# google-research/seed_rl

Hardware: NVIDIA H100
Metric: env-frames/sec (learner, device-timed) on synthetic 84x84x4 T=20 unrolls @1/2/4/8 H100 (higher is better)
Workload: dtype bf16x3 (fp32-faithful tensor-core contraction; activations stored as bf16 hi+lo pairs), f32 elsewhere

## Files before the change

seed_rl_b200/csrc/capi.cu:

```cuda
#include <vector>

#include "common.cuh"

namespace seedrl {
thread_local std::string g_last_error;
std::atomic<uint64_t> g_launch_count{0};
bool g_prof_on = false;
int g_conv_cat = PC_CONV_FWD;

struct ProfRec { int cat; cudaEvent_t e; };
static std::vector<ProfRec> g_prof;
static cudaEvent_t g_prof_start;

void prof_mark_(int cat, cudaStream_t st) {
  ProfRec r;
  r.cat = cat;
  cudaEventCreate(&r.e);
  cudaEventRecord(r.e, st);
  g_prof.push_back(r);
}
}

static const char* kProfNames[seedrl::PC_COUNT] = {
    "conv3x3_fwd", "conv3x3_dgrad", "conv3x3_wgrad", "maxpool", "sgemm", "lstm_pointwise",
    "vtrace_loss", "adam", "vtrace", "misc"};

extern "C" const char* seedrl_last_error(void) { return seedrl::g_last_error.c_str(); }
extern "C" int seedrl_abi_version(void) { return 1; }
extern "C" uint64_t seedrl_kernel_launch_count(void) {
  return seedrl::g_launch_count.load(std::memory_order_relaxed);
}

extern "C" int seedrl_profile_num_categories(void) { return seedrl::PC_COUNT; }
extern "C" const char* seedrl_profile_category_name(int i) {
// ... 34 lines not shown
```

seed_rl_b200/csrc/common.cuh:

```cuda
#pragma once
#include <cuda_runtime.h>
#include <stdint.h>
#include <stdio.h>

#include <atomic>
#include <string>

#include "../../include/seedrl_b200.h"

namespace seedrl {

extern thread_local std::string g_last_error;
extern std::atomic<uint64_t> g_launch_count;

inline int set_error(int code, const std::string& msg) {
  g_last_error = msg;
  return code;
}

#define SEEDRL_TRY(expr)                \
  do {                                  \
    const int rc__ = (expr);            \
    if (rc__ != SEEDRL_OK) return rc__; \
  } while (0)
// ... 24 lines not shown
  } while (0)

enum ProfCat { PC_CONV_FWD = 0, PC_CONV_DGRAD, PC_CONV_WGRAD, PC_POOL, PC_GEMM, PC_LSTM_PW,
               PC_LOSS, PC_ADAM, PC_VTRACE, PC_MISC, PC_COUNT };
extern bool g_prof_on;
extern int g_conv_cat;
void prof_mark_(int cat, cudaStream_t st);

inline void count_launch(int cat = PC_MISC, cudaStream_t st = 0) {
  g_launch_count.fetch_add(1, std::memory_order_relaxed);
  if (g_prof_on) prof_mark_(cat, st);
}

constexpr int kNumSMs = 132;

__host__ __device__ inline int ceil_div(int a, int b) { return (a + b - 1) / b; }
__host__ __device__ inline size_t ceil_div_sz(size_t a, size_t b) { return (a + b - 1) / b; }

__device__ __forceinline__ float warp_sum(float v) {
#pragma unroll
  for (int o = 16; o > 0; o >>= 1) v += __shfl_xor_sync(0xffffffffu, v, o);
  return v;
}
__device__ __forceinline__ float warp_max(float v) {
#pragma unroll
  for (int o = 16; o > 0; o >>= 1) v = fmaxf(v, __shfl_xor_sync(0xffffffffu, v, o));
  return v;
}

__device__ __forceinline__ float sigmoidf_(float x) { return 1.0f / (1.0f + expf(-x)); }
// ... 16 lines not shown
```

seed_rl_b200/csrc/conv_first.cu:

```cuda
#include <cuda.h>

#include <cstdlib>
#include <cstring>

#include "kernels.h"
#include "tc_common.cuh"

namespace seedrl {

constexpr int kFwThreads = 256;
constexpr int kFwCo = 16;
constexpr int kFwLanes = kFwThreads / kFwCo;

static inline int first_layer_cp(int c) { return c <= 4 ? 4 : (c <= 8 ? 8 : 16); }
static inline int fw_rows_per_band(int cp) { return cp == 16 ? 4 : 6; }
static inline size_t fw_pixels_8b(int cp, int rb, int W) { return ((size_t)(2 * rb + 3) * (W + 2) * (cp / 4) + 1) & ~(size_t)1; }
static inline size_t fw_smem(int cp, int rb, int W) {
  const int wo = (W + 1) / 2;
  return fw_pixels_8b(cp, rb, W) * 8 + (size_t)rb * wo * kFwCo * 5;
}

struct FirstWgradArgs {
  int N, H, W, C, Ho, Wo, pt, pl;
  int Lpp, PWp, RHp;
// ... 446 lines not shown
  constexpr int KT = 3 * (CP == 16 ? 48 : 4 * CP);
  const int N = a.N, H = a.H, W = a.W;
  const size_t raw_stride = TMA ? (((size_t)(2 * ROWS + 3) * W * 4) + 127) / 128 * 128 : 0;
  const size_t smem = (size_t)(CP == 16 ? 2 : 1) * (MAXB * 128 + 2 * (W + 2) + 8) * 16 +
                      (size_t)MAXB * 128 * kCpOutStride * 4 + 128 + KT * 32 * 2 + 16 * 4 + 64 + 128 + 2 * raw_stride;
  static bool attr = false;
  if (!attr) {
    SEEDRL_CUDA(cudaFuncSetAttribute(conv0pool_kernel<ROWS, CP, TMA>, cudaFuncAttributeMaxDynamicSharedMemorySize,
                                     112 * 1024));
    attr = true;
  }
  if (smem > 112 * 1024) return set_error(SEEDRL_ERR_INVALID_ARGUMENT, "conv0pool: image too wide");
  CUtensorMap tm;
  memset(&tm, 0, sizeof(tm));
  if (TMA) {
    typedef CUresult (*EncodeTiledFn)(CUtensorMap*, CUtensorMapDataType, cuuint32_t, void*, const cuuint64_t*,
                                      const cuuint64_t*, const cuuint32_t*, const cuuint32_t*, CUtensorMapInterleave,
                                      CUtensorMapSwizzle, CUtensorMapL2promotion, CUtensorMapFloatOOBfill);
    static EncodeTiledFn enc = nullptr;
    if (!enc) {
      void* q = nullptr;
      cudaDriverEntryPointQueryResult qr;
      if (cudaGetDriverEntryPoint("cuTensorMapEncodeTiled", &q, cudaEnableDefault, &qr) != cudaSuccess ||
          qr != cudaDriverEntryPointSuccess)
        return set_error(SEEDRL_ERR_INTERNAL, "cuTensorMapEncodeTiled is not available");
      enc = reinterpret_cast<EncodeTiledFn>(q);
    }
    const cuuint64_t gdim[3] = {(cuuint64_t)W, (cuuint64_t)H, (cuuint64_t)N};
    const cuuint64_t gstr[2] = {(cuuint64_t)W * 4, (cuuint64_t)H * W * 4};
    const cuuint32_t box[3] = {(cuuint32_t)W, (cuuint32_t)(2 * ROWS + 3), 1};
    const cuuint32_t estr[3] = {1, 1, 1};
    if (enc(&tm, CU_TENSOR_MAP_DATA_TYPE_UINT32, 3, const_cast<uint8_t*>(frames), gdim, gstr, box, estr,
            CU_TENSOR_MAP_INTERLEAVE_NONE, CU_TENSOR_MAP_SWIZZLE_NONE, CU_TENSOR_MAP_L2_PROMOTION_L2_128B,
            CU_TENSOR_MAP_FLOAT_OOB_FILL_NONE) != CUDA_SUCCESS)
      return set_error(SEEDRL_ERR_INTERNAL, "conv0pool: cuTensorMapEncodeTiled failed");
  }
  const int units = N * ((a.Ho + ROWS - 1) / ROWS);
  const int per_sm = ROWS == 2 ? 3 : 2;
  const int grid = units < per_sm * kNumSMs ? units : per_sm * kNumSMs;
  conv0pool_kernel<ROWS, CP, TMA><<<grid, kCpThreadsF, smem, st>>>(tm, a);
  count_launch(PC_CONV_FWD, st);
  SEEDRL_CHECK_LAUNCH();
// ... 23 lines not shown
```

seed_rl_b200/csrc/conv_planes.cu:

```cuda
#include <cuda.h>
#include <cuda_bf16.h>

#include <cstdio>
#include <cstdlib>

#include "kernels.h"
#include "tc_common.cuh"

namespace seedrl {

long long planes_positions(int N, int H, int W) {
  const long long Q = (long long)N * (H + 1) * (W + 2);
  return ((Q + 2 * (W + 2) + 2 + 256 + 127) / 128) * 128;
}
size_t planes_bytes(int N, int H, int W, int C) {
  return (size_t)planes_positions(N, H, W) * 16 * 2 * (C / 8);
}

typedef CUresult (*EncodeTiledFn)(CUtensorMap*, CUtensorMapDataType, cuuint32_t, void*, const cuuint64_t*,
                                  const cuuint64_t*, const cuuint32_t*, const cuuint32_t*,
                                  CUtensorMapInterleave, CUtensorMapSwizzle, CUtensorMapL2promotion,
                                  CUtensorMapFloatOOBfill);
static EncodeTiledFn encode_tiled_fn() {
  static EncodeTiledFn fn = nullptr;
  static bool tried = false;
  if (!tried) {
    tried = true;
    void* q = nullptr;
    cudaDriverEntryPointQueryResult qr;
    if (cudaGetDriverEntryPoint("cuTensorMapEncodeTiled", &q, cudaEnableDefault, &qr) == cudaSuccess &&
        qr == cudaDriverEntryPointSuccess)
      fn = reinterpret_cast<EncodeTiledFn>(q);
    (void)cudaGetLastError();
  }
  return fn;
}

static int g_chunk = 0;
int planes_chunk() {
  if (g_chunk == 0) {
    const char* e = getenv("SEEDRL_PLANES_CHUNK");
    g_chunk = e ? atoi(e) : 128;
    if (g_chunk != 16 && g_chunk != 32 && g_chunk != 64 && g_chunk != 128) g_chunk = 128;
  }
  return g_chunk;
}

static int make_plane_map(CUtensorMap* tm, const void* base, long long Lp, int planes, int shift,
                          int CH, int box_chunks, int box_planes) {
  EncodeTiledFn enc = encode_tiled_fn();
// ... 5 lines not shown
  const cuuint32_t box[3] = {(cuuint32_t)(2 * CH), (cuuint32_t)box_chunks, (cuuint32_t)box_planes};
  const cuuint32_t estr[3] = {1, 1, 1};
  void* addr = const_cast<char*>(reinterpret_cast<const char*>(base)) + (size_t)shift * 16;
  const CUresult r = enc(tm, CU_TENSOR_MAP_DATA_TYPE_UINT64, 3, addr, gdim, gstr, box, estr,
                         CU_TENSOR_MAP_INTERLEAVE_NONE, CU_TENSOR_MAP_SWIZZLE_NONE,
                         CU_TENSOR_MAP_L2_PROMOTION_L2_256B, CU_TENSOR_MAP_FLOAT_OOB_FILL_NONE);
  if (r != CUDA_SUCCESS) {
    char msg[128];
    snprintf(msg, sizeof msg, "cuTensorMapEncodeTiled failed (%d) Lp=%lld planes=%d shift=%d box=%dx%d", (int)r, Lp,
             planes, shift, box_chunks, box_planes);
    return set_error(SEEDRL_ERR_INTERNAL, msg);
  }
  return SEEDRL_OK;
}

__device__ __forceinline__ void mbar_expect_tx(uint64_t* bar, uint32_t bytes) {
  asm volatile("mbarrier.arrive.expect_tx.shared::cta.b64 _, [%0], %1;" ::"r"(smem_u32(bar)), "r"(bytes)
               : "memory");
}
__device__ __forceinline__ void tma_load_3d(void* dst, const CUtensorMap* tm, int c0, int c1, int c2,
                                            uint64_t* bar) {
  asm volatile(
      "cp.async.bulk.tensor.3d.shared::cluster.global.tile.mbarrier::complete_tx::bytes [%0], [%1, {%2, %3, %4}], [%5];" ::
          "r"(smem_u32(dst)),
      "l"(reinterpret_cast<uint64_t>(tm)), "r"(c0), "r"(c1), "r"(c2), "r"(smem_u32(bar))
      : "memory");
}
__device__ __forceinline__ float bf16lo(uint32_t w) { return __uint_as_float(w << 16); }
__device__ __forceinline__ float bf16hi(uint32_t w) { return __uint_as_float(w & 0xFFFF0000u); }

struct ConvpArgs {
  ConvGeom g;
  int Lp;
  int nch;
// ... 655 lines not shown
```

seed_rl_b200/csrc/gemm_tc_kernels.cu:

```cuda
#include <cstdlib>

#include "kernels.h"
#include "tc_common.cuh"

namespace seedrl {

constexpr int kGtThreads = 256;
constexpr int kGtBM = 128;
constexpr int kGtMaxBN = 128;

struct GemmTcParams {
  int M, N, K;
  const float* A; int lda;
  const float* B; int ldb;
  float* C; int ldc;
  float* ws;
  int BN;
  int kblocks_per_split;
  int vecA, vecB;
  GemmEpi e;
  int* error_flag;
  ConvGather cg;
};

// ... 43 lines not shown
      r.b = __ldg(src + 1);
    }
  }
  return r;
}
template <bool SPLIT>
__device__ __forceinline__ void store_unit(RawUnit r, bool relu, uint4* hi_dst, uint4* lo_dst) {
  if (relu) {
    r.a.x = fmaxf(r.a.x, 0.f); r.a.y = fmaxf(r.a.y, 0.f); r.a.z = fmaxf(r.a.z, 0.f); r.a.w = fmaxf(r.a.w, 0.f);
    r.b.x = fmaxf(r.b.x, 0.f); r.b.y = fmaxf(r.b.y, 0.f); r.b.z = fmaxf(r.b.z, 0.f); r.b.w = fmaxf(r.b.w, 0.f);
  }
  *hi_dst = pack8_bf16(r.a, r.b);
  if (SPLIT) *lo_dst = pack8_bf16(bf16_resid4(r.a), bf16_resid4(r.b));
}

template <int TA, int TB>
__device__ __forceinline__ void gemm_tc_mma(int bn, float* acc, uint64_t a, uint64_t b) {
  switch (bn) {
    case 16: Wgmma<16>::mma<TA, TB>(acc, a, b, 1u); break;
    case 32: Wgmma<32>::mma<TA, TB>(acc, a, b, 1u); break;
    case 48: Wgmma<48>::mma<TA, TB>(acc, a, b, 1u); break;
    case 64: Wgmma<64>::mma<TA, TB>(acc, a, b, 1u); break;
    case 80: Wgmma<80>::mma<TA, TB>(acc, a, b, 1u); break;
    case 96: Wgmma<96>::mma<TA, TB>(acc, a, b, 1u); break;
    case 112: Wgmma<112>::mma<TA, TB>(acc, a, b, 1u); break;
    default: Wgmma<128>::mma<TA, TB>(acc, a, b, 1u); break;
  }
}

template <bool TA, bool TB, bool SPLIT, int kGtBK, bool GATHER>
// ... 90 lines not shown
  {
    const int ld = BN + 4;
    float* tile = reinterpret_cast<float*>(smem_raw);
    const int w = (tid >> 5) & 3, l = tid & 31;
    const int r0 = wg * 64 + 16 * w + (l >> 2), c0 = 2 * (l & 3);
#pragma unroll
    for (int j = 0; j < kGtMaxBN / 8; ++j) {
      if (8 * j < BN) {
#pragma unroll
        for (int h = 0; h < 2; ++h)
          *reinterpret_cast<float2*>(tile + (size_t)(r0 + 8 * h) * ld + 8 * j + c0) =
              make_float2(acc[4 * j + 2 * h], acc[4 * j + 2 * h + 1]);
      }
    }
    __syncthreads();
    const bool partial = p.ws != nullptr;
    for (int i = tid; i < kGtBM * BN; i += kGtThreads) {
      const int r = i / BN, c = i - r * BN;
      const int gm = m0 + r, gn = n0 + c;
      if (gm < p.M && gn < p.N) {
        float x = tile[(size_t)r * ld + c];
        if (partial) {
          p.ws[((size_t)blockIdx.z * p.M + gm) * p.N + gn] = x;
        } else {
          if (p.e.bias) x += __ldg(p.e.bias + gn);
          if (p.e.relu) x = fmaxf(x, 0.f);
          if (p.e.mask) x = __ldg(p.e.mask + (size_t)gm * p.e.ldm + gn) > 0.f ? x : 0.f;
          float* cp = p.C + (size_t)gm * p.ldc + gn;
          *cp = p.e.accumulate ? *cp + x : x;
        }
      }
    }
  }
}

template <bool VEC>
__global__ void gemm_tc_reduce_kernel(int M, int N, int splits, const float* __restrict__ ws,
                                      float* __restrict__ C, int ldc, GemmEpi e) {
  constexpr int W = VEC ? 4 : 1;
  const int i = (blockIdx.x * blockDim.x + threadIdx.x) * W;
  if (i >= M * N) return;
  const int m = i / N, n = i - m * N;
  float x[W];
#pragma unroll
  for (int j = 0; j < W; ++j) x[j] = 0.f;
  const size_t plane = (size_t)M * N;
#pragma unroll 4
// ... 73 lines not shown

bool conv_gather_setup(const void* x, int u8, int N, int H, int W, int C, int K, int S, ConvGather* g) {
  const int Ho = (H - K) / S + 1, Wo = (W - K) / S + 1, KC = K * C;
  if (Ho < 2 || Wo < 2 || KC < 8 || (KC & 7)) return false;
  if ((long long)N * Ho * Wo >= (1ll << 31)) return false;
  if (u8 ? (((W * C) & 7) || ((S * C) & 7) || (reinterpret_cast<uintptr_t>(x) & 7))
         : ((C & 3) || (reinterpret_cast<uintptr_t>(x) & 15)))
    return false;
  g->x = x; g->u8 = u8; g->H = H; g->W = W; g->C = C; g->S = S; g->Ho = Ho; g->Wo = Wo; g->KC = KC;
  fast_div_setup((unsigned int)Wo, &g->wo_mul, &g->wo_sh);
  fast_div_setup((unsigned int)Ho, &g->ho_mul, &g->ho_sh);
  fast_div_setup((unsigned int)KC, &g->kc_mul, &g->kc_sh);
  return true;
}

int gemm_tc(bool ta, bool tb, int split, int M, int N, int K, const float* A, int lda, const float* B,
            int ldb, float* C, int ldc, const GemmEpi& e, float* ws, size_t ws_bytes, int* err,
            cudaStream_t st, const ConvGather* cg) {
  if (M <= 0 || N <= 0) return SEEDRL_OK;
  SEEDRL_CHECK_ARG(!cg || (!tb && ((ta ? M : K) & 7) == 0), "gathered operand: tb or a ragged kernel row");
  GemmTcParams p;
  if (cg) p.cg = *cg; else p.cg = ConvGather{};
  p.M = M; p.N = N; p.K = K; p.A = A; p.lda = lda; p.B = B; p.ldb = ldb; p.C = C; p.ldc = ldc;
  p.e = e; p.error_flag = err;
  const int n16 = ((N + 15) / 16) * 16;
  const int BK = g_gemm_bk;
  int bn = kGtMaxBN;
  if (bn > n16) bn = n16;
  const int nkb_all = ceil_div(K, BK);
  const int kb256 = 256 / BK;
  while (bn > 64 && ceil_div(M, kGtBM) * ceil_div(N, bn) * (nkb_all >= kb256 ? nkb_all / (kb256 / 2) : 1) < kNumSMs)
    bn >>= 1;
  p.BN = ((bn + 15) / 16) * 16;
// ... 5 lines not shown
  int splits = 1;
  static const int waves = getenv("SEEDRL_GEMM_WAVES") ? atoi(getenv("SEEDRL_GEMM_WAVES")) : 1;
  while (tiles * splits < waves * kNumSMs && nkb / (splits * 2) >= 128 / BK &&
         (size_t)(splits * 2) * M * N * sizeof(float) <= ws_bytes && ws)
    splits *= 2;
  p.kblocks_per_split = ceil_div(nkb, splits);
  splits = ceil_div(nkb, p.kblocks_per_split);
  p.ws = splits > 1 ? ws : nullptr;
  const int S = split ? 2 : 1;
  const size_t a_un = ta ? (size_t)(kGtBM / 8) * (BK + 1) : (size_t)(BK / 8) * (kGtBM + 1);
  const size_t b_un = tb ? (size_t)(BK / 8) * (p.BN + 1) : (size_t)(p.BN / 8) * (BK + 1);
  size_t smem = (size_t)2 * S * (a_un + b_un) * 16;
  const size_t epi = (size_t)kGtBM * (p.BN + 4) * 4;
  if (smem < epi) smem = epi;
  dim3 grid(ceil_div(N, p.BN), ceil_div(M, kGtBM), splits);
#define SEEDRL_GT_LAUNCH2(TA_, TB_, SP_, BK_, G_)                                               \
  do {                                                                                          \
    static bool attr = false;                                                                   \
    if (!attr) {                                                                                \
      SEEDRL_CUDA(cudaFuncSetAttribute(gemm_tc_kernel<TA_, TB_, SP_, BK_, G_>,                  \
                                       cudaFuncAttributeMaxDynamicSharedMemorySize, 200 * 1024)); \
      attr = true;                                                                              \
    }                                                                                           \
    gemm_tc_kernel<TA_, TB_, SP_, BK_, G_><<<grid, kGtThreads, smem, st>>>(p);                  \
  } while (0)
#define SEEDRL_GT_LAUNCH1(TA_, TB_, SP_, BK_)                                                   \
  do {                                                                                          \
    if (cg && !(TB_)) SEEDRL_GT_LAUNCH2(TA_, false, SP_, BK_, true);                            \
    else SEEDRL_GT_LAUNCH2(TA_, TB_, SP_, BK_, false);                                          \
  } while (0)
// ... 5 lines not shown
  } while (0)
  if (split) {
    if (!ta && !tb) SEEDRL_GT_LAUNCH(false, false, true);
    else if (ta && !tb) SEEDRL_GT_LAUNCH(true, false, true);
    else if (!ta && tb) SEEDRL_GT_LAUNCH(false, true, true);
    else SEEDRL_GT_LAUNCH(true, true, true);
  } else {
    if (!ta && !tb) SEEDRL_GT_LAUNCH(false, false, false);
    else if (ta && !tb) SEEDRL_GT_LAUNCH(true, false, false);
    else if (!ta && tb) SEEDRL_GT_LAUNCH(false, true, false);
    else SEEDRL_GT_LAUNCH(true, true, false);
  }
#undef SEEDRL_GT_LAUNCH
#undef SEEDRL_GT_LAUNCH1
#undef SEEDRL_GT_LAUNCH2
  count_launch(PC_GEMM, st);
  SEEDRL_CHECK_LAUNCH();
  if (splits > 1) {
    if ((N & 3) == 0 && splits >= 16)
      gemm_tc_reduce_wide_kernel<<<ceil_div(M * N / 4, 32), 256, 0, st>>>(M, N, splits, ws, C, ldc, e);
    else if ((N & 3) == 0)
      gemm_tc_reduce_kernel<true><<<ceil_div(M * N / 4, 256), 256, 0, st>>>(M, N, splits, ws, C, ldc, e);
    else
      gemm_tc_reduce_kernel<false><<<ceil_div(M * N, 256), 256, 0, st>>>(M, N, splits, ws, C, ldc, e);
    count_launch(PC_GEMM, st);
    SEEDRL_CHECK_LAUNCH();
  }
  return SEEDRL_OK;
}

}
```

seed_rl_b200/csrc/kernels.h:

```cpp
#pragma once
#include "common.cuh"

namespace seedrl {

enum { IN_F32 = 0, IN_RELU = 1, IN_U8 = 2 };

struct ConvGeom {
  int N, H, W;
  int PW;
  int RH;
  long long Q;
  unsigned int pw_mul, rh_mul;
  int pw_sh, rh_sh;
};

__host__ __device__ inline void fast_div_setup(unsigned int d, unsigned int* mul, int* sh) {
  int l = 1;
  while ((1u << l) < d) ++l;
  *mul = (unsigned int)(((1ULL << (31 + l)) + d - 1) / d);
  *sh = l - 1;
}
__host__ __device__ __forceinline__ unsigned int fast_div(unsigned int n, unsigned int mul, int sh) {
#ifdef __CUDA_ARCH__
  return __umulhi(n, mul) >> sh;
// ... 130 lines not shown
size_t gemm_tc_workspace_bytes();
struct ConvGather {
  const void* x;
  int u8;
  int H, W, C, S, Ho, Wo;
  int KC;
  unsigned int wo_mul, ho_mul, kc_mul;
  int wo_sh, ho_sh, kc_sh;
};
bool conv_gather_setup(const void* x, int u8, int N, int H, int W, int C, int K, int S, ConvGather* g);
void gemm_tc_set_gather(int on);
bool gemm_tc_gather_enabled();
int gemm_tc(bool ta, bool tb, int split, int M, int N, int K, const float* A, int lda, const float* B,
            int ldb, float* C, int ldc, const GemmEpi& e, float* ws, size_t ws_bytes, int* err,
            cudaStream_t st, const ConvGather* cg = nullptr);
int fill(size_t n, float* p, float v, cudaStream_t st);

int lstm_forward_tiled(int H, int T1, int B, const float* U, const uint8_t* done, float* z, const float* h0,
                       const float* c0, float* hs, float* cs, float* hp, unsigned int* counter, int* err,
                       cudaStream_t st);
int lstm_backward_tiled(int H, int T1, int B, const float* U, const uint8_t* done, const float* gates,
                        const float* cs, const float* c0, const float* dhs, float* dz, unsigned int* counter,
                        int* err, cudaStream_t st);

int lstm_forward_tc(int H, int T1, int B, const float* U, const uint8_t* done, float* z, const float* h0,
                    const float* c0, float* hs, float* cs, float* hp, unsigned int* counter, int* err,
                    cudaStream_t st);
int lstm_backward_tc(int H, int T1, int B, const float* U, const uint8_t* done, const float* gates,
                     const float* cs, const float* c0, const float* dhs, float* dz, unsigned int* counter,
                     int* err, cudaStream_t st);
// ... 3 lines not shown
```

seed_rl_b200/csrc/net.cu:

```cuda
#include "schedule.h"

namespace seedrl {

constexpr int kHidden = 256;

struct ConvLayer {
  int cin, cout;
  int w, b;
};
struct Stack {
  int hin, win, cin, c, hout, wout;
  ConvLayer conv, r00, r01, r10, r11;
};

}

struct seedrl_net {
  seedrl_net_config cfg;
  seedrl::ParamTable params;
  size_t logical_params;
  int p_base_w, p_base_b, p_pol_w, p_pol_b;
  seedrl::Core core;
  std::vector<seedrl::Stack> stacks;
  seedrl::StridedConv sh[2];
// ... 697 lines not shown
                                          const void* x, const float* dy, float* dw, float* db,
                                          float* partial, size_t partial_bytes,
                                          seedrl_stream_t stream) {
  return conv3x3_wgrad(cin, cout, in_mode, N, H, W, x, dy, dw, db, partial, partial_bytes,
                       (cudaStream_t)stream);
}
extern "C" int seedrl_debug_maxpool(int backward, int N, int H, int W, int C, const float* x_or_dy,
                                    float* y_or_dx, uint8_t* idx, seedrl_stream_t stream) {
  if (backward) return maxpool3s2_backward(N, H, W, C, x_or_dy, idx, y_or_dx, (cudaStream_t)stream);
  return maxpool3s2_forward(N, H, W, C, x_or_dy, y_or_dx, idx, (cudaStream_t)stream);
}
extern "C" int seedrl_debug_gemm_tc(int ta, int tb, int split, int M, int N, int K, const float* A, int lda,
                                    const float* B, int ldb, float* C, int ldc, const float* bias,
                                    const float* mask, int ldm, int relu, int accumulate, int a_relu,
                                    float* ws, size_t ws_bytes, int* error_flag, seedrl_stream_t stream) {
  SEEDRL_CHECK_ARG(M >= 1 && N >= 1 && K >= 1 && A && B && C, "bad arguments");
  GemmEpi e{bias, mask, ldm, relu, accumulate, a_relu};
  return gemm_tc(ta != 0, tb != 0, split, M, N, K, A, lda, B, ldb, C, ldc, e, ws, ws_bytes, error_flag,
                 (cudaStream_t)stream);
}

extern "C" int seedrl_debug_sgemm(int ta, int tb, int M, int N, int K, const float* A, int lda,
                                  const float* B, int ldb, float* C, int ldc, const float* bias,
                                  const float* mask, int ldm, int relu, int accumulate, int a_relu,
                                  seedrl_stream_t stream) {
  GemmEpi e{bias, mask, ldm, relu, accumulate, a_relu};
  return sgemm(ta != 0, tb != 0, M, N, K, A, lda, B, ldb, C, ldc, e, (cudaStream_t)stream);
}

extern "C" int seedrl_debug_set_gemm_gather(int on) {
  gemm_tc_set_gather(on);
  return SEEDRL_OK;
// ... 118 lines not shown
```

seed_rl_b200/csrc/tc_common.cuh:

```cuda
#pragma once
#include <cuda_bf16.h>
#include <stdint.h>

namespace seedrl {

__device__ __forceinline__ uint32_t smem_u32(const void* p) {
  return static_cast<uint32_t>(__cvta_generic_to_shared(p));
}

__device__ __forceinline__ bool elect_one() {
  uint32_t pred;
  asm volatile(
      "{\n\t.reg .pred P;\n\t"
      "elect.sync _|P, 0xffffffff;\n\t"
      "selp.u32 %0, 1, 0, P;\n\t}\n"
      : "=r"(pred));
  return pred != 0;
}

__device__ __forceinline__ uint64_t gmma_desc(uint32_t addr, uint32_t lbo_bytes, uint32_t sbo_bytes) {
  uint64_t d = 0;
  d |= (uint64_t)((addr & 0x3FFFFu) >> 4);
  d |= (uint64_t)((lbo_bytes >> 4) & 0x3FFFu) << 16;
  d |= (uint64_t)((sbo_bytes >> 4) & 0x3FFFu) << 32;
// ... 44 lines not shown
        "selp.u32 %0, 1, 0, p;\n\t}\n"
        : "=r"(done)
        : "r"(smem_u32(bar)), "r"(parity)
        : "memory");
    if (!done && ++spins > (1 << 22)) return false;
  }
  return true;
}
__device__ __forceinline__ void mbar_init(uint64_t* bar, int count) {
  asm volatile("mbarrier.init.shared::cta.b64 [%0], %1;" ::"r"(smem_u32(bar)), "r"(count));
}
__device__ __forceinline__ void mbar_arrive(uint64_t* bar) {
  asm volatile("{\n\t.reg .b64 st;\n\tmbarrier.arrive.shared::cta.b64 st, [%0];\n\t}\n" ::"r"(smem_u32(bar))
               : "memory");
}

template <>
struct Wgmma<16> {
  template <int TA, int TB>
  __device__ __forceinline__ static void mma(float* d, uint64_t a, uint64_t b, uint32_t scale_d) {
    asm volatile(
        "{\n\t.reg .pred p;\n\tsetp.ne.b32 p, %10, 0;\n\t"
        "wgmma.mma_async.sync.aligned.m64n16k16.f32.bf16.bf16 {%0, %1, %2, %3, %4, %5, %6, %7}, %8, %9, p, 1, 1, %11, %12;\n\t}\n"
        : "+f"(d[0]), "+f"(d[1]), "+f"(d[2]), "+f"(d[3]), "+f"(d[4]), "+f"(d[5]), "+f"(d[6]), "+f"(d[7])
        : "l"(a), "l"(b), "r"(scale_d), "n"(TA), "n"(TB));
  }
};

template <>
struct Wgmma<24> {
// ... 154 lines not shown
```

seed_rl_b200/csrc/vtrace_kernels.cu:

```cuda
#include <cuda.h>
#include <math.h>

#include <type_traits>

#include "common.cuh"

namespace seedrl {

template <int CH>
__global__ void __launch_bounds__(128)
vtrace_kernel(int T, int B, const float* __restrict__ tlp, const float* __restrict__ blp,
              const float* __restrict__ disc, const float* __restrict__ rew,
              const float* __restrict__ val, const float* __restrict__ boot,
              float clip_rho, float clip_pg, float lambda_, int has_clip_rho,
              int has_clip_pg, float* __restrict__ vs, float* __restrict__ pg) {
  const int b = blockIdx.x * blockDim.x + threadIdx.x;
  if (b >= B) return;
  float acc = 0.f;
  const float bootv = boot[b];
  float vs_next = bootv, v_next = bootv;
  int t_hi = T;
  while (t_hi > 0) {
    const int t_lo = t_hi - CH > 0 ? t_hi - CH : 0;
    float a_t[CH], a_b[CH], a_d[CH], a_r[CH], a_v[CH];
// ... 842 lines not shown
  const size_t rows = (size_t)T * BB;
  return (3 * (size_t)stream_tile_stride_f(T, A, BB) + 9 * rows + (size_t)(T + 1) * BB + rows + 32) * 4 + 3 * 8 + 128;
}

static int num_sms() {
  static int n = 0;
  if (n == 0) {
    int dev = 0;
    if (cudaGetDevice(&dev) != cudaSuccess ||
        cudaDeviceGetAttribute(&n, cudaDevAttrMultiProcessorCount, dev) != cudaSuccess || n <= 0)
      n = kNumSMs;
  }
  return n;
}

typedef CUresult (*EncodeTiledFn)(CUtensorMap*, CUtensorMapDataType, cuuint32_t, void*, const cuuint64_t*,
                                  const cuuint64_t*, const cuuint32_t*, const cuuint32_t*,
                                  CUtensorMapInterleave, CUtensorMapSwizzle, CUtensorMapL2promotion,
                                  CUtensorMapFloatOOBfill);
static EncodeTiledFn encode_tiled() {
  static EncodeTiledFn fn = nullptr;
  static bool tried = false;
  if (!tried) {
    tried = true;
    void* q = nullptr;
    cudaDriverEntryPointQueryResult qr;
    if (cudaGetDriverEntryPoint("cuTensorMapEncodeTiled", &q, cudaEnableDefault, &qr) == cudaSuccess &&
        qr == cudaDriverEntryPointSuccess)
      fn = reinterpret_cast<EncodeTiledFn>(q);
    (void)cudaGetLastError();
  }
  return fn;
}
static bool make_tile_map(CUtensorMap* tm, const float* base, int T1, int T, int B, int A, int BB) {
  const cuuint64_t gdim[2] = {(cuuint64_t)B * A, (cuuint64_t)T1};
  const cuuint64_t gstr[1] = {(cuuint64_t)B * A * sizeof(float)};
  const cuuint32_t box[2] = {(cuuint32_t)(BB * A), (cuuint32_t)T};
  const cuuint32_t estr[2] = {1, 1};
  return encode_tiled()(tm, CU_TENSOR_MAP_DATA_TYPE_FLOAT32, 2, const_cast<float*>(base), gdim, gstr, box,
                        estr, CU_TENSOR_MAP_INTERLEAVE_NONE, CU_TENSOR_MAP_SWIZZLE_NONE,
                        CU_TENSOR_MAP_L2_PROMOTION_L2_256B, CU_TENSOR_MAP_FLOAT_OOB_FILL_NONE) == CUDA_SUCCESS;
}

static int pick_stream(const LossParams& p, int forced_bb, int* threads, size_t* smem_bytes) {
  const int T = p.T, B = p.B, A = p.A;
  auto aligned16 = [](const void* q) { return (reinterpret_cast<uintptr_t>(q) & 15) == 0; };
  if (!aligned16(p.ll) || !aligned16(p.bl) || !aligned16(p.dlogits)) return 0;
  if (T > 256 || (((size_t)B * A) & 3) != 0 || !encode_tiled()) return 0;
  for (int pass = 0; pass < 2; ++pass)
  for (int BB = 16; BB >= 2; BB >>= 1) {
    if (forced_bb > 1 && BB != forced_bb) continue;
    if (B % BB != 0 || ((BB * A) & 3) != 0 || BB * A > 256) continue;
    if (B / BB < num_sms()) continue;
    const size_t bytes = stream_smem_bytes(T, A, BB);
    if (bytes > kStreamSmemMax) continue;
    if (pass == 0 && forced_bb <= 1 && 2 * (bytes + 2048 + 1024) > (size_t)228 * 1024) continue;
    const int rows = T * BB;
    const int rounds = ceil_div(rows, kStreamThreadsMax);
    int th = ceil_div(ceil_div(rows, rounds), 32) * 32;
    if (th < 128) th = 128;
    if ((T + 1) * BB > kStreamRounds * th) continue;
    *threads = th;
    *smem_bytes = bytes;
// ... 167 lines not shown
```

Baseline: 197,800.

## Add warp-specialized TMA-fed producer/consumer pipeline for tensor-core GEMM

Adds a new GEMM kernel in which a dedicated producer warp streams fp32 A/B tiles into a multi-stage shared-memory ring via TMA with mbarrier full/empty signalling. Two consumer warpgroups convert each stage to bf16 hi/lo and issue wgmma, overlapping global loads with conversion and MMA. The epilogue is batched so loads of bias, mask and the accumulator are issued before the stores. The new path is the default for non-gathered, vector-aligned BK=32 GEMMs, and the old staged kernel stays reachable through a split flag bit. This is meant to hide load latency, at the cost of host-side tensor-map encoding on every launch and a smaller k-step (16) per stage.

```diff
diff --git a/seed_rl_b200/csrc/capi.cu b/seed_rl_b200/csrc/capi.cu
--- a/seed_rl_b200/csrc/capi.cu
+++ b/seed_rl_b200/csrc/capi.cu
@@ -18,6 +18,21 @@
   cudaEventCreate(&r.e);
   cudaEventRecord(r.e, st);
   g_prof.push_back(r);
+}
+
+EncodeTiledFn encode_tiled_fn() {
+  static EncodeTiledFn fn = nullptr;
+  static bool tried = false;
+  if (!tried) {
+    tried = true;
+    void* q = nullptr;
+    cudaDriverEntryPointQueryResult qr;
+    if (cudaGetDriverEntryPoint("cuTensorMapEncodeTiled", &q, cudaEnableDefault, &qr) == cudaSuccess &&
+        qr == cudaDriverEntryPointSuccess)
+      fn = reinterpret_cast<EncodeTiledFn>(q);
+    (void)cudaGetLastError();
+  }
+  return fn;
 }
 }
 
diff --git a/seed_rl_b200/csrc/common.cuh b/seed_rl_b200/csrc/common.cuh
--- a/seed_rl_b200/csrc/common.cuh
+++ b/seed_rl_b200/csrc/common.cuh
@@ -1,4 +1,5 @@
 #pragma once
+#include <cuda.h>
 #include <cuda_runtime.h>
 #include <stdint.h>
 #include <stdio.h>
@@ -62,6 +63,12 @@
 
 constexpr int kNumSMs = 132;
 
+typedef CUresult (*EncodeTiledFn)(CUtensorMap*, CUtensorMapDataType, cuuint32_t, void*, const cuuint64_t*,
+                                  const cuuint64_t*, const cuuint32_t*, const cuuint32_t*,
+                                  CUtensorMapInterleave, CUtensorMapSwizzle, CUtensorMapL2promotion,
+                                  CUtensorMapFloatOOBfill);
+EncodeTiledFn encode_tiled_fn();
+
 __host__ __device__ inline int ceil_div(int a, int b) { return (a + b - 1) / b; }
 __host__ __device__ inline size_t ceil_div_sz(size_t a, size_t b) { return (a + b - 1) / b; }
 
diff --git a/seed_rl_b200/csrc/conv_first.cu b/seed_rl_b200/csrc/conv_first.cu
--- a/seed_rl_b200/csrc/conv_first.cu
+++ b/seed_rl_b200/csrc/conv_first.cu
@@ -484,18 +484,8 @@
   CUtensorMap tm;
   memset(&tm, 0, sizeof(tm));
   if (TMA) {
-    typedef CUresult (*EncodeTiledFn)(CUtensorMap*, CUtensorMapDataType, cuuint32_t, void*, const cuuint64_t*,
-                                      const cuuint64_t*, const cuuint32_t*, const cuuint32_t*, CUtensorMapInterleave,
-                                      CUtensorMapSwizzle, CUtensorMapL2promotion, CUtensorMapFloatOOBfill);
-    static EncodeTiledFn enc = nullptr;
-    if (!enc) {
-      void* q = nullptr;
-      cudaDriverEntryPointQueryResult qr;
-      if (cudaGetDriverEntryPoint("cuTensorMapEncodeTiled", &q, cudaEnableDefault, &qr) != cudaSuccess ||
-          qr != cudaDriverEntryPointSuccess)
-        return set_error(SEEDRL_ERR_INTERNAL, "cuTensorMapEncodeTiled is not available");
-      enc = reinterpret_cast<EncodeTiledFn>(q);
-    }
+    const EncodeTiledFn enc = encode_tiled_fn();
+    if (!enc) return set_error(SEEDRL_ERR_INTERNAL, "cuTensorMapEncodeTiled is not available");
     const cuuint64_t gdim[3] = {(cuuint64_t)W, (cuuint64_t)H, (cuuint64_t)N};
     const cuuint64_t gstr[2] = {(cuuint64_t)W * 4, (cuuint64_t)H * W * 4};
     const cuuint32_t box[3] = {(cuuint32_t)W, (cuuint32_t)(2 * ROWS + 3), 1};
diff --git a/seed_rl_b200/csrc/conv_planes.cu b/seed_rl_b200/csrc/conv_planes.cu
--- a/seed_rl_b200/csrc/conv_planes.cu
+++ b/seed_rl_b200/csrc/conv_planes.cu
@@ -15,25 +15,6 @@
 }
 size_t planes_bytes(int N, int H, int W, int C) {
   return (size_t)planes_positions(N, H, W) * 16 * 2 * (C / 8);
-}
-
-typedef CUresult (*EncodeTiledFn)(CUtensorMap*, CUtensorMapDataType, cuuint32_t, void*, const cuuint64_t*,
-                                  const cuuint64_t*, const cuuint32_t*, const cuuint32_t*,
-                                  CUtensorMapInterleave, CUtensorMapSwizzle, CUtensorMapL2promotion,
-                                  CUtensorMapFloatOOBfill);
-static EncodeTiledFn encode_tiled_fn() {
-  static EncodeTiledFn fn = nullptr;
-  static bool tried = false;
-  if (!tried) {
-    tried = true;
-    void* q = nullptr;
-    cudaDriverEntryPointQueryResult qr;
-    if (cudaGetDriverEntryPoint("cuTensorMapEncodeTiled", &q, cudaEnableDefault, &qr) == cudaSuccess &&
-        qr == cudaDriverEntryPointSuccess)
-      fn = reinterpret_cast<EncodeTiledFn>(q);
-    (void)cudaGetLastError();
-  }
-  return fn;
 }
 
 static int g_chunk = 0;
@@ -69,10 +50,6 @@
   return SEEDRL_OK;
 }
 
-__device__ __forceinline__ void mbar_expect_tx(uint64_t* bar, uint32_t bytes) {
-  asm volatile("mbarrier.arrive.expect_tx.shared::cta.b64 _, [%0], %1;" ::"r"(smem_u32(bar)), "r"(bytes)
-               : "memory");
-}
 __device__ __forceinline__ void tma_load_3d(void* dst, const CUtensorMap* tm, int c0, int c1, int c2,
                                             uint64_t* bar) {
   asm volatile(
diff --git a/seed_rl_b200/csrc/gemm_tc_kernels.cu b/seed_rl_b200/csrc/gemm_tc_kernels.cu
--- a/seed_rl_b200/csrc/gemm_tc_kernels.cu
+++ b/seed_rl_b200/csrc/gemm_tc_kernels.cu
@@ -81,6 +81,49 @@
   if (SPLIT) *lo_dst = pack8_bf16(bf16_resid4(r.a), bf16_resid4(r.b));
 }
 
+constexpr int kEpiBatch = 8;
+template <int NT>
+__device__ __forceinline__ void store_tile(const GemmTcParams& p, const float* tile, int ld, int BN, int m0,
+                                           int n0, int tid) {
+  const bool partial = p.ws != nullptr;
+  for (int i0 = tid; i0 < kGtBM * BN; i0 += NT * kEpiBatch) {
+    float x[kEpiBatch], mk[kEpiBatch], cv[kEpiBatch];
+    size_t off[kEpiBatch];
+    bool in[kEpiBatch];
+#pragma unroll
+    for (int u = 0; u < kEpiBatch; ++u) {
+      const int i = i0 + u * NT;
+      const int r = i / BN, c = i - r * BN;
+      const int gm = m0 + r, gn = n0 + c;
+      in[u] = i < kGtBM * BN && gm < p.M && gn < p.N;
+      x[u] = 0.f; mk[u] = 1.f; cv[u] = 0.f; off[u] = 0;
+      if (in[u]) {
+        x[u] = tile[(size_t)r * ld + c];
+        if (partial) {
+          off[u] = ((size_t)blockIdx.z * p.M + gm) * p.N + gn;
+        } else {
+          off[u] = (size_t)gm * p.ldc + gn;
+          if (p.e.bias) x[u] += __ldg(p.e.bias + gn);
+          if (p.e.mask) mk[u] = __ldg(p.e.mask + (size_t)gm * p.e.ldm + gn);
+          if (p.e.accumulate) cv[u] = p.C[off[u]];
+        }
+      }
+    }
+#pragma unroll
+    for (int u = 0; u < kEpiBatch; ++u) {
+      if (!in[u]) continue;
+      float v = x[u];
+      if (partial) {
+        p.ws[off[u]] = v;
+      } else {
+        if (p.e.relu) v = fmaxf(v, 0.f);
+        if (p.e.mask) v = mk[u] > 0.f ? v : 0.f;
+        p.C[off[u]] = p.e.accumulate ? cv[u] + v : v;
+      }
+    }
+  }
+}
+
 template <int TA, int TB>
 __device__ __forceinline__ void gemm_tc_mma(int bn, float* acc, uint64_t a, uint64_t b) {
   switch (bn) {
@@ -201,23 +244,219 @@
       }
     }
     __syncthreads();
-    const bool partial = p.ws != nullptr;
-    for (int i = tid; i < kGtBM * BN; i += kGtThreads) {
-      const int r = i / BN, c = i - r * BN;
-      const int gm = m0 + r, gn = n0 + c;
-      if (gm < p.M && gn < p.N) {
-        float x = tile[(size_t)r * ld + c];
-        if (partial) {
-          p.ws[((size_t)blockIdx.z * p.M + gm) * p.N + gn] = x;
-        } else {
-          if (p.e.bias) x += __ldg(p.e.bias + gn);
-          if (p.e.relu) x = fmaxf(x, 0.f);
-          if (p.e.mask) x = __ldg(p.e.mask + (size_t)gm * p.e.ldm + gn) > 0.f ? x : 0.f;
-          float* cp = p.C + (size_t)gm * p.ldc + gn;
-          *cp = p.e.accumulate ? *cp + x : x;
-        }
-      }
-    }
+    store_tile<kGtThreads>(p, tile, ld, BN, m0, n0, tid);
+  }
+}
+
+constexpr int kGpConsumers = 256;
+constexpr int kGpThreads = kGpConsumers + 32;
+constexpr int kGpKS = 16;
+constexpr int kGpConv = 3;
+constexpr int kGpMaxRaw = 8;
+constexpr uint32_t kGpSmemBudget = 113 * 1024;
+
+template <bool TA, bool TB, bool SPLIT, int BN>
+struct GpLayout {
+  static constexpr int S = SPLIT ? 2 : 1;
+  static constexpr uint32_t a_ps = TA ? kGpKS + 1 : kGtBM + 1;
+  static constexpr uint32_t a_units = TA ? (kGtBM / 8) * a_ps : (kGpKS / 8) * a_ps;
+  static constexpr uint32_t b_ps = TB ? BN + 1 : kGpKS + 1;
+  static constexpr uint32_t b_units = TB ? (kGpKS / 8) * b_ps : (BN / 8) * b_ps;
+  static constexpr uint32_t conv_bytes = S * (a_units + b_units) * 16;
+  static constexpr uint32_t a_raw = kGtBM * kGpKS * 4, raw_bytes = a_raw + BN * kGpKS * 4;
+  static constexpr int NS0 = (int)((kGpSmemBudget - kGpConv * conv_bytes - 2 * kGpMaxRaw * 8) / raw_bytes);
+  static constexpr int NS = NS0 < kGpMaxRaw ? NS0 : kGpMaxRaw;
+  static constexpr uint32_t bar_off = NS * raw_bytes + kGpConv * conv_bytes;
+  static constexpr uint32_t epi_bytes = kGtBM * (BN + 4) * 4;
+  static constexpr uint32_t smem = (bar_off + 2 * NS * 8) > epi_bytes ? bar_off + 2 * NS * 8 : epi_bytes;
+  static_assert(NS >= 3, "the raw ring must hold three stages");
+};
+
+__device__ __forceinline__ void tma_load_2d(void* dst, const CUtensorMap* tm, int c0, int c1, uint64_t* bar) {
+  asm volatile(
+      "cp.async.bulk.tensor.2d.shared::cluster.global.tile.mbarrier::complete_tx::bytes [%0], [%1, {%2, %3}], [%4];" ::
+          "r"(smem_u32(dst)), "l"(reinterpret_cast<uint64_t>(tm)), "r"(c0), "r"(c1), "r"(smem_u32(bar))
+      : "memory");
+}
+__device__ __forceinline__ void consumer_sync() { asm volatile("bar.sync 1, %0;" ::"n"(kGpConsumers) : "memory"); }
+__device__ __forceinline__ RawUnit lds_unit(const float* p, int i) {
+  const int f = (i >> 2) & 1;
+  const float4 x = *reinterpret_cast<const float4*>(p + 4 * f);
+  const float4 y = *reinterpret_cast<const float4*>(p + 4 - 4 * f);
+  RawUnit r;
+  r.a = f ? y : x;
+  r.b = f ? x : y;
+  return r;
+}
+
+template <bool TA, bool TB, bool SPLIT, int BN>
+__global__ void __launch_bounds__(kGpThreads, 2)
+gemm_tc_tma_kernel(const __grid_constant__ CUtensorMap tm_a, const __grid_constant__ CUtensorMap tm_b,
+                   const GemmTcParams p) {
+  using Lay = GpLayout<TA, TB, SPLIT, BN>;
+  constexpr int NS = Lay::NS;
+  extern __shared__ __align__(128) uint8_t smem_raw[];
+  uint64_t* full = reinterpret_cast<uint64_t*>(smem_raw + Lay::bar_off);
+  uint64_t* empty = full + NS;
+  const int tid = threadIdx.x, warp = tid >> 5;
+  const int m0 = blockIdx.y * kGtBM, n0 = blockIdx.x * BN;
+  const int kb0 = blockIdx.z * p.kblocks_per_split;
+  const int nsteps = min(p.kblocks_per_split, (p.K + 31) / 32 - kb0) * (32 / kGpKS);
+  if (tid == 0) {
+    for (int s = 0; s < NS; ++s) {
+      mbar_init(full + s, 1);
+      mbar_init(empty + s, kGpConsumers / 32);
+    }
+    asm volatile("fence.mbarrier_init.release.cluster;" ::: "memory");
+    asm volatile("prefetch.tensormap [%0];" ::"l"(reinterpret_cast<uint64_t>(&tm_a)) : "memory");
+    asm volatile("prefetch.tensormap [%0];" ::"l"(reinterpret_cast<uint64_t>(&tm_b)) : "memory");
+  }
+  __syncthreads();
+  bool timed_out = false;
+
+  if (warp == kGpConsumers / 32) {
+    if (elect_one()) {
+      for (int j = 0; j < nsteps; ++j) {
+        const int s = j % NS;
+        if (j >= NS && !mbar_wait_bounded(empty + s, (uint32_t)(((j / NS) - 1) & 1))) { timed_out = true; break; }
+        uint8_t* st = smem_raw + (size_t)s * Lay::raw_bytes;
+        const int k = kb0 * 32 + j * kGpKS;
+        mbar_expect_tx(full + s, Lay::raw_bytes);
+        if (TA) tma_load_2d(st, &tm_a, m0, k, full + s); else tma_load_2d(st, &tm_a, k, m0, full + s);
+        if (TB) tma_load_2d(st + Lay::a_raw, &tm_b, k, n0, full + s);
+        else    tma_load_2d(st + Lay::a_raw, &tm_b, n0, k, full + s);
+      }
+    }
+    __syncwarp();
+    if (timed_out && p.error_flag) atomicExch(p.error_flag, 1);
+    return;
+  }
+
+  const int wg = tid >> 7, t = tid & 127;
+  const bool a_relu = p.e.a_relu != 0;
+  const uint32_t a_wg = TA ? (uint32_t)wg * 8u * Lay::a_ps * 16u : (uint32_t)wg * 64u * 16u;
+  float acc[BN / 2];
+#pragma unroll
+  for (int i = 0; i < BN / 2; ++i) acc[i] = 0.f;
+  wgmma_fence_acc<BN / 2>(acc);
+
+  for (int j = 0; j < nsteps; ++j) {
+    const int s = j % NS;
+    if (!timed_out && !mbar_wait_bounded(full + s, (uint32_t)((j / NS) & 1))) timed_out = true;
+    if (j >= 2) wgmma_wait<1>();
+    const float* ra = reinterpret_cast<const float*>(smem_raw + (size_t)s * Lay::raw_bytes);
+    const float* rb = ra + Lay::a_raw / 4;
+    uint4* sA = reinterpret_cast<uint4*>(smem_raw + (size_t)NS * Lay::raw_bytes + (size_t)(j % kGpConv) * Lay::conv_bytes);
+    uint4* sB = sA + Lay::S * Lay::a_units;
+    {
+      uint32_t o;
+      RawUnit r;
+      if (!TA) {
+        const int row = 64 * wg + (t >> 1), kg = t & 1;
+        r = lds_unit(ra + row * kGpKS + kg * 8, t);
+        o = (uint32_t)kg * Lay::a_ps + row;
+      } else {
+        const int k = t >> 3, mg = 8 * wg + (t & 7);
+        r = lds_unit(ra + k * kGtBM + mg * 8, t);
+        o = (uint32_t)mg * Lay::a_ps + k;
+      }
+      store_unit<SPLIT>(r, a_relu, sA + o, sA + Lay::a_units + o);
+    }
+#pragma unroll
+    for (int u = tid; u < BN * kGpKS / 8; u += kGpConsumers) {
+      uint32_t o;
+      RawUnit r;
+      if (TB) {
+        const int n = u >> 1, kg = u & 1;
+        r = lds_unit(rb + n * kGpKS + kg * 8, u);
+        o = (uint32_t)kg * Lay::b_ps + n;
+      } else {
+        const int k = u / (BN / 8), ng = u % (BN / 8);
+        r = lds_unit(rb + k * BN + ng * 8, u);
+        o = (uint32_t)ng * Lay::b_ps + k;
+      }
+      store_unit<SPLIT>(r, false, sB + o, sB + Lay::b_units + o);
+    }
+    __syncwarp();
+    if ((tid & 31) == 0) mbar_arrive(empty + s);
+    asm volatile("fence.proxy.async.shared::cta;" ::: "memory");
+    consumer_sync();
+    wgmma_fence();
+    const uint32_t a_addr = smem_u32(sA) + a_wg, b_addr = smem_u32(sB);
+    const uint64_t da = TA ? gmma_desc(a_addr, 128u, Lay::a_ps * 16u) : gmma_desc(a_addr, Lay::a_ps * 16u, 128u);
+    const uint64_t db = TB ? gmma_desc(b_addr, Lay::b_ps * 16u, 128u) : gmma_desc(b_addr, 128u, Lay::b_ps * 16u);
+    Wgmma<BN>::template mma<TA ? 1 : 0, TB ? 0 : 1>(acc, da, db, 1u);
+    if (SPLIT) {
+      Wgmma<BN>::template mma<TA ? 1 : 0, TB ? 0 : 1>(acc, da + Lay::a_units, db, 1u);
+      Wgmma<BN>::template mma<TA ? 1 : 0, TB ? 0 : 1>(acc, da, db + Lay::b_units, 1u);
+    }
+    wgmma_commit();
+  }
+  wgmma_wait<0>();
+  wgmma_fence_acc<BN / 2>(acc);
+  if (timed_out && p.error_flag) atomicExch(p.error_flag, 1);
+
+  consumer_sync();
+  {
+    constexpr int ld = BN + 4;
+    float* tile = reinterpret_cast<float*>(smem_raw);
+    const int w = (tid >> 5) & 3, l = tid & 31;
+    const int r0 = wg * 64 + 16 * w + (l >> 2), c0 = 2 * (l & 3);
+#pragma unroll
+    for (int j = 0; j < BN / 8; ++j) {
+#pragma unroll
+      for (int h = 0; h < 2; ++h)
+        *reinterpret_cast<float2*>(tile + (size_t)(r0 + 8 * h) * ld + 8 * j + c0) =
+            make_float2(acc[4 * j + 2 * h], acc[4 * j + 2 * h + 1]);
+    }
+    consumer_sync();
+    store_tile<kGpConsumers>(p, tile, ld, BN, m0, n0, tid);
+  }
+}
+
+static int make_gemm_map(CUtensorMap* tm, const float* base, int rows, int cols, int ld, int box_c, int box_r) {
+  const EncodeTiledFn enc = encode_tiled_fn();
+  if (!enc) return set_error(SEEDRL_ERR_INTERNAL, "cuTensorMapEncodeTiled is not available");
+  const cuuint64_t gdim[2] = {(cuuint64_t)cols, (cuuint64_t)rows};
+  const cuuint64_t gstr[1] = {(cuuint64_t)ld * sizeof(float)};
+  const cuuint32_t box[2] = {(cuuint32_t)box_c, (cuuint32_t)box_r};
+  const cuuint32_t estr[2] = {1, 1};
+  if (enc(tm, CU_TENSOR_MAP_DATA_TYPE_FLOAT32, 2, const_cast<float*>(base), gdim, gstr, box, estr,
+          CU_TENSOR_MAP_INTERLEAVE_NONE, CU_TENSOR_MAP_SWIZZLE_NONE, CU_TENSOR_MAP_L2_PROMOTION_L2_256B,
+          CU_TENSOR_MAP_FLOAT_OOB_FILL_NONE) != CUDA_SUCCESS)
+    return set_error(SEEDRL_ERR_INTERNAL, "gemm_tc: cuTensorMapEncodeTiled failed");
+  return SEEDRL_OK;
+}
+
+template <bool TA, bool TB, bool SPLIT, int BN>
+static int launch_gemm_tma(const GemmTcParams& p, dim3 grid, cudaStream_t st) {
+  using Lay = GpLayout<TA, TB, SPLIT, BN>;
+  alignas(64) CUtensorMap tm_a, tm_b;
+  if (TA) SEEDRL_TRY(make_gemm_map(&tm_a, p.A, p.K, p.M, p.lda, kGtBM, kGpKS));
+  else    SEEDRL_TRY(make_gemm_map(&tm_a, p.A, p.M, p.K, p.lda, kGpKS, kGtBM));
+  if (TB) SEEDRL_TRY(make_gemm_map(&tm_b, p.B, p.N, p.K, p.ldb, kGpKS, BN));
+  else    SEEDRL_TRY(make_gemm_map(&tm_b, p.B, p.K, p.N, p.ldb, BN, kGpKS));
+  static bool attr = false;
+  if (!attr) {
+    SEEDRL_CUDA(cudaFuncSetAttribute(gemm_tc_tma_kernel<TA, TB, SPLIT, BN>,
+                                     cudaFuncAttributeMaxDynamicSharedMemorySize, (int)Lay::smem));
+    attr = true;
+  }
+  gemm_tc_tma_kernel<TA, TB, SPLIT, BN><<<grid, kGpThreads, Lay::smem, st>>>(tm_a, tm_b, p);
+  return SEEDRL_OK;
+}
+
+template <bool TA, bool TB, bool SPLIT>
+static int launch_gemm_tma_bn(const GemmTcParams& p, dim3 grid, cudaStream_t st) {
+  switch (p.BN) {
+    case 16: return launch_gemm_tma<TA, TB, SPLIT, 16>(p, grid, st);
+    case 32: return launch_gemm_tma<TA, TB, SPLIT, 32>(p, grid, st);
+    case 48: return launch_gemm_tma<TA, TB, SPLIT, 48>(p, grid, st);
+    case 64: return launch_gemm_tma<TA, TB, SPLIT, 64>(p, grid, st);
+    case 80: return launch_gemm_tma<TA, TB, SPLIT, 80>(p, grid, st);
+    case 96: return launch_gemm_tma<TA, TB, SPLIT, 96>(p, grid, st);
+    case 112: return launch_gemm_tma<TA, TB, SPLIT, 112>(p, grid, st);
+    default: return launch_gemm_tma<TA, TB, SPLIT, 128>(p, grid, st);
   }
 }
 
@@ -321,9 +560,9 @@
   return true;
 }
 
-int gemm_tc(bool ta, bool tb, int split, int M, int N, int K, const float* A, int lda, const float* B,
-            int ldb, float* C, int ldc, const GemmEpi& e, float* ws, size_t ws_bytes, int* err,
-            cudaStream_t st, const ConvGather* cg) {
+static int gemm_tc_run(bool ta, bool tb, int split, int M, int N, int K, const float* A, int lda, const float* B,
+                       int ldb, float* C, int ldc, const GemmEpi& e, float* ws, size_t ws_bytes, int* err,
+                       cudaStream_t st, const ConvGather* cg, bool allow_tma) {
   if (M <= 0 || N <= 0) return SEEDRL_OK;
   SEEDRL_CHECK_ARG(!cg || (!tb && ((ta ? M : K) & 7) == 0), "gathered operand: tb or a ragged kernel row");
   GemmTcParams p;
@@ -359,6 +598,21 @@
   const size_t epi = (size_t)kGtBM * (p.BN + 4) * 4;
   if (smem < epi) smem = epi;
   dim3 grid(ceil_div(N, p.BN), ceil_div(M, kGtBM), splits);
+  if (!cg && p.vecA && p.vecB && BK == 32 && allow_tma) {
+    int rc;
+    if (split) {
+      if (!ta && !tb) rc = launch_gemm_tma_bn<false, false, true>(p, grid, st);
+      else if (ta && !tb) rc = launch_gemm_tma_bn<true, false, true>(p, grid, st);
+      else if (!ta && tb) rc = launch_gemm_tma_bn<false, true, true>(p, grid, st);
+      else rc = launch_gemm_tma_bn<true, true, true>(p, grid, st);
+    } else {
+      if (!ta && !tb) rc = launch_gemm_tma_bn<false, false, false>(p, grid, st);
+      else if (ta && !tb) rc = launch_gemm_tma_bn<true, false, false>(p, grid, st);
+      else if (!ta && tb) rc = launch_gemm_tma_bn<false, true, false>(p, grid, st);
+      else rc = launch_gemm_tma_bn<true, true, false>(p, grid, st);
+    }
+    SEEDRL_TRY(rc);
+  } else {
 #define SEEDRL_GT_LAUNCH2(TA_, TB_, SP_, BK_, G_)                                               \
   do {                                                                                          \
     static bool attr = false;                                                                   \
@@ -394,6 +648,7 @@
 #undef SEEDRL_GT_LAUNCH
 #undef SEEDRL_GT_LAUNCH1
 #undef SEEDRL_GT_LAUNCH2
+  }
   count_launch(PC_GEMM, st);
   SEEDRL_CHECK_LAUNCH();
   if (splits > 1) {
@@ -409,4 +664,16 @@
   return SEEDRL_OK;
 }
 
-}
+int gemm_tc(bool ta, bool tb, int split, int M, int N, int K, const float* A, int lda, const float* B, int ldb,
+            float* C, int ldc, const GemmEpi& e, float* ws, size_t ws_bytes, int* err, cudaStream_t st,
+            const ConvGather* cg) {
+  return gemm_tc_run(ta, tb, split, M, N, K, A, lda, B, ldb, C, ldc, e, ws, ws_bytes, err, st, cg, true);
+}
+
+int gemm_tc_staged(bool ta, bool tb, int split, int M, int N, int K, const float* A, int lda, const float* B,
+                   int ldb, float* C, int ldc, const GemmEpi& e, float* ws, size_t ws_bytes, int* err,
+                   cudaStream_t st) {
+  return gemm_tc_run(ta, tb, split, M, N, K, A, lda, B, ldb, C, ldc, e, ws, ws_bytes, err, st, nullptr, false);
+}
+
+}
diff --git a/seed_rl_b200/csrc/kernels.h b/seed_rl_b200/csrc/kernels.h
--- a/seed_rl_b200/csrc/kernels.h
+++ b/seed_rl_b200/csrc/kernels.h
@@ -168,6 +168,9 @@
 int gemm_tc(bool ta, bool tb, int split, int M, int N, int K, const float* A, int lda, const float* B,
             int ldb, float* C, int ldc, const GemmEpi& e, float* ws, size_t ws_bytes, int* err,
             cudaStream_t st, const ConvGather* cg = nullptr);
+int gemm_tc_staged(bool ta, bool tb, int split, int M, int N, int K, const float* A, int lda, const float* B,
+                   int ldb, float* C, int ldc, const GemmEpi& e, float* ws, size_t ws_bytes, int* err,
+                   cudaStream_t st);
 int fill(size_t n, float* p, float v, cudaStream_t st);
 
 int lstm_forward_tiled(int H, int T1, int B, const float* U, const uint8_t* done, float* z, const float* h0,
diff --git a/seed_rl_b200/csrc/net.cu b/seed_rl_b200/csrc/net.cu
--- a/seed_rl_b200/csrc/net.cu
+++ b/seed_rl_b200/csrc/net.cu
@@ -735,8 +735,11 @@
                                     const float* B, int ldb, float* C, int ldc, const float* bias,
                                     const float* mask, int ldm, int relu, int accumulate, int a_relu,
                                     float* ws, size_t ws_bytes, int* error_flag, seedrl_stream_t stream) {
-  SEEDRL_CHECK_ARG(M >= 1 && N >= 1 && K >= 1 && A && B && C, "bad arguments");
+  SEEDRL_CHECK_ARG(M >= 1 && N >= 1 && K >= 1 && A && B && C && split >= 0 && split <= 3, "bad arguments");
   GemmEpi e{bias, mask, ldm, relu, accumulate, a_relu};
+  if (split & 2)
+    return gemm_tc_staged(ta != 0, tb != 0, split & 1, M, N, K, A, lda, B, ldb, C, ldc, e, ws, ws_bytes,
+                          error_flag, (cudaStream_t)stream);
   return gemm_tc(ta != 0, tb != 0, split, M, N, K, A, lda, B, ldb, C, ldc, e, ws, ws_bytes, error_flag,
                  (cudaStream_t)stream);
 }
diff --git a/seed_rl_b200/csrc/tc_common.cuh b/seed_rl_b200/csrc/tc_common.cuh
--- a/seed_rl_b200/csrc/tc_common.cuh
+++ b/seed_rl_b200/csrc/tc_common.cuh
@@ -82,6 +82,10 @@
   asm volatile("{\n\t.reg .b64 st;\n\tmbarrier.arrive.shared::cta.b64 st, [%0];\n\t}\n" ::"r"(smem_u32(bar))
                : "memory");
 }
+__device__ __forceinline__ void mbar_expect_tx(uint64_t* bar, uint32_t bytes) {
+  asm volatile("mbarrier.arrive.expect_tx.shared::cta.b64 _, [%0], %1;" ::"r"(smem_u32(bar)), "r"(bytes)
+               : "memory");
+}
 
 template <>
 struct Wgmma<16> {
diff --git a/seed_rl_b200/csrc/vtrace_kernels.cu b/seed_rl_b200/csrc/vtrace_kernels.cu
--- a/seed_rl_b200/csrc/vtrace_kernels.cu
+++ b/seed_rl_b200/csrc/vtrace_kernels.cu
@@ -880,30 +880,12 @@
   return n;
 }
 
-typedef CUresult (*EncodeTiledFn)(CUtensorMap*, CUtensorMapDataType, cuuint32_t, void*, const cuuint64_t*,
-                                  const cuuint64_t*, const cuuint32_t*, const cuuint32_t*,
-                                  CUtensorMapInterleave, CUtensorMapSwizzle, CUtensorMapL2promotion,
-                                  CUtensorMapFloatOOBfill);
-static EncodeTiledFn encode_tiled() {
-  static EncodeTiledFn fn = nullptr;
-  static bool tried = false;
-  if (!tried) {
-    tried = true;
-    void* q = nullptr;
-    cudaDriverEntryPointQueryResult qr;
-    if (cudaGetDriverEntryPoint("cuTensorMapEncodeTiled", &q, cudaEnableDefault, &qr) == cudaSuccess &&
-        qr == cudaDriverEntryPointSuccess)
-      fn = reinterpret_cast<EncodeTiledFn>(q);
-    (void)cudaGetLastError();
-  }
-  return fn;
-}
 static bool make_tile_map(CUtensorMap* tm, const float* base, int T1, int T, int B, int A, int BB) {
   const cuuint64_t gdim[2] = {(cuuint64_t)B * A, (cuuint64_t)T1};
   const cuuint64_t gstr[1] = {(cuuint64_t)B * A * sizeof(float)};
   const cuuint32_t box[2] = {(cuuint32_t)(BB * A), (cuuint32_t)T};
   const cuuint32_t estr[2] = {1, 1};
-  return encode_tiled()(tm, CU_TENSOR_MAP_DATA_TYPE_FLOAT32, 2, const_cast<float*>(base), gdim, gstr, box,
+  return encode_tiled_fn()(tm, CU_TENSOR_MAP_DATA_TYPE_FLOAT32, 2, const_cast<float*>(base), gdim, gstr, box,
                         estr, CU_TENSOR_MAP_INTERLEAVE_NONE, CU_TENSOR_MAP_SWIZZLE_NONE,
                         CU_TENSOR_MAP_L2_PROMOTION_L2_256B, CU_TENSOR_MAP_FLOAT_OOB_FILL_NONE) == CUDA_SUCCESS;
 }
@@ -912,7 +894,7 @@
   const int T = p.T, B = p.B, A = p.A;
   auto aligned16 = [](const void* q) { return (reinterpret_cast<uintptr_t>(q) & 15) == 0; };
   if (!aligned16(p.ll) || !aligned16(p.bl) || !aligned16(p.dlogits)) return 0;
-  if (T > 256 || (((size_t)B * A) & 3) != 0 || !encode_tiled()) return 0;
+  if (T > 256 || (((size_t)B * A) & 3) != 0 || !encode_tiled_fn()) return 0;
   for (int pass = 0; pass < 2; ++pass)
   for (int BB = 16; BB >= 2; BB >>= 1) {
     if (forced_bb > 1 && BB != forced_bb) continue;
```

After: 200,000 (median of 6 runs). +1.1%, better.
